# noveens/reviews4rec

Hardware: AMD Instinct MI355X
Metric: train ratings/sec (higher is better)
Workload: dtype f32

## Files before the change

include/r4r.h:

```cpp
#ifndef R4R_H
#define R4R_H

#include <stddef.h>
#include <stdint.h>

#ifdef __cplusplus
extern "C" {
#endif

#define R4R_OK 0
#define R4R_ERR_ARG (-1)
#define R4R_ERR_LAUNCH (-2)
#define R4R_ERR_WORKSPACE (-3)

int r4r_version(void);
const char *r4r_last_error(void);

size_t r4r_textcnn_ws_bytes(int64_t N, int T, int E, int F, int64_t V);
int r4r_textcnn_fwd(const float *table, int64_t V, const int64_t *idx,
                    const float *conv_w, const float *conv_b,
                    float *pooled, int32_t *argmax,
                    void *ws, size_t ws_bytes,
                    int64_t N, int T, int E, int F, void *stream);

int r4r_conv_algo(int requested, int64_t N, int T, int E, int F);

int r4r_textcnn_algo(int requested);

int r4r_conv_pick(int E, int T, int64_t docs, int64_t rows, int64_t V);

int r4r_gemm_math(int mode, float table_maxabs, float weight_maxabs);

int r4r_gemm_form(int balanced);

int r4r_textcnn_wgrad(const float *table, int64_t V, const int64_t *idx,
                      const float *g_pooled, const int32_t *argmax,
                      float *d_conv_w, float *d_conv_b,
                      void *ws, size_t ws_bytes,
                      int64_t N, int T, int E, int F, void *stream);

int r4r_linear_fwd(const float *x, const float *w, const float *b, float *y,
                   int64_t N, int n_in, int n_out, int relu, void *stream);
size_t r4r_linear_bwd_ws_bytes(int64_t N, int n_in, int n_out);
int r4r_linear_bwd(const float *x, const float *w, const float *y, const float *g_y,
                   float *g_x, float *g_w, float *g_b, void *ws, size_t ws_bytes,
                   int64_t N, int n_in, int n_out, int relu, void *stream);

int r4r_dropout_fwd(const float *x, float *y, float *mult, int64_t n, float p,
                    uint64_t seed, uint64_t offset, uint64_t *offset_dev, void *stream);
int r4r_counter_add(uint64_t *counter, uint64_t delta, void *stream);
int r4r_mul(const float *a, const float *b, float *out, int64_t n, void *stream);
int r4r_add(const float *a, const float *b, float *out, int64_t n, void *stream);

int r4r_fm_fwd(const float *x, const float *V, const float *lin_w, const float *lin_b,
               float *out, int64_t N, int n, int k, void *stream);
int r4r_fm_bwd(const float *x, const float *V, const float *lin_w, const float *g_out,
// ... 45 lines not shown
                      float weight_decay, int64_t step, void *stream);
int r4r_adam_gathered_guarded(float *p, const float *gathered, int world, float *g_sum, float *m, float *v,
                              int64_t numel, float lr, double beta1, double beta2, float eps,
                              float weight_decay, int64_t step, const uint32_t *abort_word, void *stream);

int r4r_peer_segment_create(int64_t bytes, void **ptr, uint8_t *handle);
int r4r_peer_segment_open(const uint8_t *handle, void **ptr);
int r4r_peer_segment_close(void *ptr);
int r4r_peer_segment_destroy(void *ptr);
int r4r_peer_push(const float *src, int64_t numel, const uint64_t *peer_dst, const uint64_t *peer_flags,
                  uint32_t *arrive, int rank, int world, uint32_t epoch, const uint32_t *wait_flags,
                  uint32_t *timed_out, double timeout_s, void *stream);
int r4r_peer_wait(const uint32_t *flags, int world, uint32_t epoch, uint32_t *timed_out, double timeout_s, void *stream);


#define R4R_CONV_AUTO 0
#define R4R_CONV_DIRECT 1
#define R4R_CONV_PROJECT 2
int r4r_deepconn_nparam(void);
int r4r_deepconn_layout(int E, int L, int64_t *offsets, int64_t *sizes, int64_t *total);
size_t r4r_deepconn_ws_bytes(int64_t B, int T, int E, int L, int64_t V);
size_t r4r_deepconn_ws_mult_offset(int64_t B, int T, int E, int L, int64_t V);
size_t r4r_deepconn_ws_count_offset(int64_t B, int T, int E, int L, int64_t V, int tower, int buffer);
int r4r_deepconn_step(const float *table, int64_t V, const int64_t *user_idx, const int64_t *item_idx,
                      const float *y, float *flat_p, float *flat_g,
                      float *pred, float *se, float *sse_accum,
                      void *ws, size_t ws_bytes,
                      int64_t B, int T, int E, int L,
                      float dropout_p, int training, uint64_t seed, uint64_t offset,
                      float inv_denom, int conv_algo, int token_buffer, int tokens_ready,
                      const int64_t *next_user_idx, const int64_t *next_item_idx,
                      float *flat_m, float *flat_v, float lr, double beta1, double beta2, float eps,
                      float weight_decay, int64_t adam_step, void *stream);
int r4r_deepconn_tokens(const int64_t *user_idx, const int64_t *item_idx, void *ws, size_t ws_bytes,
                        int64_t B, int T, int E, int L, int64_t V, int conv_algo, int token_buffer,
                        int discard, void *stream);

#define R4R_TIMING_TEXTCNN_FWD 0
#define R4R_TIMING_TEXTCNN_WGRAD 1
#define R4R_TIMING_ADAM 2
#define R4R_TIMING_PROJ_GEMM 3
#define R4R_TIMING_PROJ_GATHER 4
#define R4R_TIMING_SLOTS 8
int r4r_timing_enable(int slot_mask);
int r4r_timing_read(int slot, double *total_ms, int64_t *count, int reset);

// ... 365 lines not shown
```

reviews4rec_amd/csrc/engine.hip:

```cpp
#include <stdlib.h>

#include "trace_device.h"
#include "textcnn.h"
#include "wgrad_device.h"
#include "tokens_device.h"
#include "adam_device.h"

namespace r4r {

constexpr int F_CONV = 100;
constexpr int FM_K = 8;
constexpr int MAX_L = 128;

enum { P_UCW = 0, P_UCB, P_UFW, P_UFB, P_ICW, P_ICB, P_IFW, P_IFB, P_FMV, P_FMLW, P_FMLB, P_GB, P_COUNT };

struct Layout {
    int64_t off[P_COUNT], size[P_COUNT], total;
};

static Layout make_layout(int E, int L) {
    Layout lay;
    const int64_t sz[P_COUNT] = {(int64_t)F_CONV * 3 * E, F_CONV, (int64_t)L * F_CONV, L,
                                 (int64_t)F_CONV * 3 * E, F_CONV, (int64_t)L * F_CONV, L,
                                 (int64_t)2 * L * FM_K, 2 * L, 1, 1};
// ... 1 lines not shown
    for (int i = 0; i < P_COUNT; ++i) {
        lay.off[i] = o;
        lay.size[i] = sz[i];
        o += (sz[i] + 31) & ~(int64_t)31;
    }
    lay.total = o;
    return lay;
}

struct HeadArgs {
    const float *pmax[2]; const int *parg[2];
    const float *fc_w[2]; const float *fc_b[2];
    const float *V, *lin_w, *lin_b, *gbias;
    const float *y;
    float *pooled[2]; int *argmax[2];
    float *g_pooled[2];
    float *mult;
    float *x, *s, *g, *gz;
    float *pred, *se;
    int64_t B;
    int L, tiles, training, want_grad;
    float p_drop, inv_denom;
    uint64_t seed, offset;
};


constexpr int HEAD_MAX_TILES = 8;

#define SEL2(arr, s) ((s) ? (arr)[1] : (arr)[0])
HEAD_TRACE_DEFINE(r4r_debug_dc_head_trace)
template <int ML>
__global__ __launch_bounds__(256) void deepconn_head_wg_kernel(HeadArgs a) {
    HEAD_STAMP(0)
    constexpr int N2 = 2 * ML, PARTS = 256 / N2;
    __shared__ float sw[2][ML][F_CONV + 1];
    __shared__ float sfb[N2], slw[N2], sz[N2];
    __shared__ float sV[N2][FM_K];
    __shared__ float sp[2][F_CONV + 4];
    __shared__ float red[N2][PARTS + 1];
    const int tid = threadIdx.x, lane = tid & 63, w = tid >> 6;
    const int64_t b = blockIdx.x;
    const int L = a.L, n = 2 * L;
    const float lin_b0 = a.lin_b[0], gbias0 = a.gbias[0], yb = a.y ? a.y[b] : 0.f;

    constexpr int FQ = F_CONV / 4;
    typedef float hq4 __attribute__((ext_vector_type(4)));
    constexpr int WREGS = (2 * ML * FQ + 255) / 256;
    hq4 wreg[WREGS];
    const int wtot = 2 * L * FQ;
#pragma unroll
    for (int k = 0; k < WREGS; ++k) {
        const int i = min(tid + 256 * k, wtot - 1);
        const int t = i >= L * FQ;
        wreg[k] = *reinterpret_cast<const hq4 *>(SEL2(a.fc_w, t) + 4 * (i - t * L * FQ));
    }
    const int tn = min(tid, n - 1);
    const float fbreg = SEL2(a.fc_b, tn >= L)[tn - (tn >= L ? L : 0)];
    const float lwreg = a.lin_w[tn];
    constexpr int VREGS = (N2 * FM_K + 255) / 256;
    float vreg[VREGS];
#pragma unroll
    for (int k = 0; k < VREGS; ++k) vreg[k] = a.V[min(tid + 256 * k, n * FM_K - 1)];

    {
        const int t = w >> 1, f = lane + 64 * (w & 1), fc = min(f, F_CONV - 1);
        float best = -INFINITY;
        int bp = -1;
        if (a.tiles <= HEAD_MAX_TILES) {
            float v[HEAD_MAX_TILES];
            int pp[HEAD_MAX_TILES];
#pragma unroll
            for (int k = 0; k < HEAD_MAX_TILES; ++k) {
                const size_t o = ((size_t)b * a.tiles + min(k, a.tiles - 1)) * NP + fc;
                v[k] = SEL2(a.pmax, t)[o];
                pp[k] = SEL2(a.parg, t)[o];
            }
#pragma unroll
            for (int k = 0; k < HEAD_MAX_TILES; ++k)
                if (v[k] > best) { best = v[k]; bp = pp[k]; }
        } else {
            for (int k0 = 0; k0 < a.tiles; k0 += HEAD_MAX_TILES) {
                float v[HEAD_MAX_TILES];
                int pp[HEAD_MAX_TILES];
#pragma unroll
                for (int k = 0; k < HEAD_MAX_TILES; ++k) {
// ... 195 lines not shown
        float t = 0.f;
#pragma unroll
        for (int r = 0; r < HG_ROWS; ++r) t += red[r][ox];
        switch (which) {
            case 0: a.g_fc_w[0][local] = t; break;
            case 1: a.g_fc_b[0][local] = t; break;
            case 2: a.g_fc_w[1][local] = t; break;
            case 3: a.g_fc_b[1][local] = t; break;
            case 4: a.g_V[local] = t; break;
            case 5: a.g_lin_w[local] = t; break;
            case 6: a.g_lin_b[0] = t; break;
            case 7: a.g_gb[0] = t; break;
            default: if (a.sse_accum) a.sse_accum[0] += t; break;
        }
    }
}

BWD_TRACE_DEFINE(r4r_debug_dc_bwd_trace)
struct DcBackwardArgs {
    WgradArgs w;
    HeadGradArgs h;
    int hg_blocks;
    TokenArgs nx;
};
__global__ __launch_bounds__(WG_THREADS, 8) void deepconn_backward_kernel(DcBackwardArgs) {
    const DcBackwardArgs &A = kernel_args<DcBackwardArgs>();
    const WgradArgs &w = A.w;
    const HeadGradArgs &h = A.h;
    const TokenArgs &nx = A.nx;
    const int hg_blocks = A.hg_blocks;
    BWD_STAMP(0, wall_clock64())
    BWD_STAMP(2, (unsigned long long)blockIdx.z + 1)
    if (blockIdx.z == 1 || blockIdx.z == 2) {
        wgrad_block(w, blockIdx.x, blockIdx.y, blockIdx.z - 1);
    } else if (blockIdx.z == 0) {
        for (int blk = blockIdx.y * gridDim.x + blockIdx.x; blk < hg_blocks; blk += gridDim.x * gridDim.y) {
            head_grad_block(h, blk);
            __syncthreads();
        }
    } else {
        token_mark_block(nx, blockIdx.y * gridDim.x + blockIdx.x, gridDim.x * gridDim.y, WG_THREADS);
    }
#ifdef R4R_TRACE
    __syncthreads();
#endif
    BWD_STAMP(1, wall_clock64())
}

constexpr int RED_THREADS = 256;
struct FusedAdam {
    float *p, *m, *v;
    const float *g;
    int64_t lo[2], hi[2];
    AdamScalars s;
    int on;
};
__global__ __launch_bounds__(RED_THREADS) void deepconn_reduce_kernel(WgradArgs w, int red_blocks, int comp_blocks,
                                                                      TokenArgs nx, FusedAdam opt) {
    const int bx = blockIdx.x;
    if (bx < red_blocks) {
        const WgradTower &tw = w.t[blockIdx.y];
        const int nw = w.F * 3 * w.E;
        const int i = bx * RED_THREADS + threadIdx.x;
        const float *gp0 = i < nw ? tw.d_w + i : (i < nw + w.F ? tw.d_b + (i - nw) : nullptr);
// ... 14 lines not shown
            float P = opt.p[o], M = opt.m[o], V = opt.v[o];
            adam_elem(P, opt.g[o], M, V, opt.s);
            opt.p[o] = P; opt.m[o] = M; opt.v[o] = V;
        }
    }
}

__global__ void sse_only_kernel(const float *__restrict__ se, float *__restrict__ accum, int64_t B) {
    __shared__ float red[256];
    float s = 0.f;
    for (int64_t i = threadIdx.x; i < B; i += 256) s += se[i];
    red[threadIdx.x] = s;
    __syncthreads();
    for (int off = 128; off > 0; off >>= 1) {
        if ((int)threadIdx.x < off) red[threadIdx.x] += red[threadIdx.x + off];
        __syncthreads();
    }
    if (threadIdx.x == 0) accum[0] += red[0];
}

struct StepWs {
    float *wp[2], *pmax[2]; int *parg[2];
    int *flags[2][2], *slot[2][2], *list[2][2], *count[2][2]; float *ptab[2];
    float *pooled[2]; int *argmax[2]; float *g_pooled[2];
    float *mult, *x, *s, *g, *gz;
    float *part_w[2], *part_b[2];
    size_t bytes;
};

static StepWs carve(void *ws, int64_t B, int T, int E, int L, int64_t V) {
    StepWs w;
    char *p = static_cast<char *>(ws);
    auto take = [&](size_t nbytes) { char *r = p; p += align256(nbytes); return r; };
    const size_t tiles128 = (size_t)(T + 2 + 127) / 128;
    const int ns = textcnn_wgrad_splits(B);
    for (int t = 0; t < 2; ++t) {
        w.wp[t] = reinterpret_cast<float *>(take(textcnn_wp_floats(E) * 4));
        w.pmax[t] = reinterpret_cast<float *>(take((size_t)B * tiles128 * NP * 4));
        w.parg[t] = reinterpret_cast<int *>(take((size_t)B * tiles128 * NP * 4));
        w.pooled[t] = reinterpret_cast<float *>(take((size_t)B * F_CONV * 4));
        w.argmax[t] = reinterpret_cast<int *>(take((size_t)B * F_CONV * 4));
        w.g_pooled[t] = reinterpret_cast<float *>(take((size_t)B * F_CONV * 4));
        w.part_w[t] = reinterpret_cast<float *>(take((size_t)ns * F_CONV * 3 * E * 4));
        w.part_b[t] = reinterpret_cast<float *>(take((size_t)ns * F_CONV * 4));
        for (int bf = 0; bf < 2; ++bf) {
            w.flags[bf][t] = reinterpret_cast<int *>(take((size_t)(V + 4) * 4));
            w.slot[bf][t] = reinterpret_cast<int *>(take((size_t)(V + 4) * 4));
            w.list[bf][t] = reinterpret_cast<int *>(take((size_t)proj_row_capacity(B, T, V) * 4));
            w.count[bf][t] = reinterpret_cast<int *>(take(256));
        }
        w.ptab[t] = reinterpret_cast<float *>(take(proj_ptab_floats(B, T, V) * 4));
    }
    w.mult = reinterpret_cast<float *>(take((size_t)B * 2 * L * 4));
    w.x = reinterpret_cast<float *>(take((size_t)B * 2 * L * 4));
    w.gz = reinterpret_cast<float *>(take((size_t)B * 2 * L * 4));
    w.s = reinterpret_cast<float *>(take((size_t)B * FM_K * 4));
    w.g = reinterpret_cast<float *>(take((size_t)B * 4));
    w.bytes = (size_t)(p - static_cast<char *>(ws));
    return w;
}

}

using namespace r4r;

extern "C" int r4r_deepconn_nparam(void) { return P_COUNT; }

extern "C" int r4r_deepconn_layout(int E, int L, int64_t *offsets, int64_t *sizes, int64_t *total) {
    R4R_REQUIRE(E > 0 && L > 0 && L <= MAX_L && offsets && sizes && total, "deepconn_layout: bad arguments");
    const Layout lay = make_layout(E, L);
    for (int i = 0; i < P_COUNT; ++i) { offsets[i] = lay.off[i]; sizes[i] = lay.size[i]; }
    *total = lay.total;
    return R4R_OK;
}

extern "C" size_t r4r_deepconn_ws_bytes(int64_t B, int T, int E, int L, int64_t V) {
    if (B < 0 || T <= 0 || E <= 0 || L <= 0 || V <= 0) return 0;
    return carve(nullptr, B, T, E, L, V).bytes;
}

extern "C" size_t r4r_deepconn_ws_mult_offset(int64_t B, int T, int E, int L, int64_t V) {
    char base[1];
    const StepWs w = carve(base, B, T, E, L, V);
    return (size_t)(reinterpret_cast<char *>(w.mult) - base);
}

extern "C" size_t r4r_deepconn_ws_count_offset(int64_t B, int T, int E, int L, int64_t V, int tower, int buffer) {
    char base[1];
    const StepWs w = carve(base, B, T, E, L, V);
    return (size_t)(reinterpret_cast<char *>(w.count[buffer & 1][tower & 1]) - base);
}

extern "C" int r4r_deepconn_tokens(const int64_t *user_idx, const int64_t *item_idx, void *ws, size_t ws_bytes,
                                   int64_t B, int T, int E, int L, int64_t V, int conv_algo, int token_buffer,
                                   int discard, void *stream) {
    R4R_REQUIRE(user_idx && item_idx && ws, "deepconn_tokens: null pointer");
    R4R_REQUIRE(token_buffer == 0 || token_buffer == 1, "deepconn_tokens: token_buffer must be 0 or 1");
    if (ws_bytes < r4r_deepconn_ws_bytes(B, T, E, L, V)) {
        set_error("deepconn_tokens: workspace %zu < %zu bytes", ws_bytes, r4r_deepconn_ws_bytes(B, T, E, L, V));
        return R4R_ERR_WORKSPACE;
    }
    if (B == 0 || textcnn_pick_algo(conv_algo, B, T, E, F_CONV) != R4R_CONV_PROJECT) return R4R_OK;
    const StepWs w = carve(ws, B, T, E, L, V);
    if (discard) {
        for (int t = 0; t < 2; ++t) (void)hipMemsetAsync(w.count[token_buffer][t], 0, sizeof(int), as_stream(stream));
        return check_launch("deepconn_tokens(discard)");
    }
    ProjTower pt[2];
    const int64_t *idx[2] = {user_idx, item_idx};
    for (int t = 0; t < 2; ++t) {
        pt[t] = ProjTower{};
        pt[t].idx = idx[t];
        pt[t].flags = w.flags[token_buffer][t]; pt[t].slot = w.slot[token_buffer][t];
        pt[t].list = w.list[token_buffer][t]; pt[t].count = w.count[token_buffer][t];
    }
    return textcnn_proj_tokens_launch(V, pt, 2, B, T, false, as_stream(stream));
}

extern "C" int r4r_deepconn_step(const float *table, int64_t V, const int64_t *user_idx, const int64_t *item_idx,
                                 const float *y, float *flat_p, float *flat_g,
                                 float *pred, float *se, float *sse_accum,
                                 void *ws, size_t ws_bytes,
                                 int64_t B, int T, int E, int L,
                                 float dropout_p, int training, uint64_t seed, uint64_t offset,
                                 float inv_denom, int conv_algo, int token_buffer, int tokens_ready,
                                 const int64_t *next_user_idx, const int64_t *next_item_idx,
                                 float *flat_m, float *flat_v, float lr, double beta1, double beta2, float eps,
                                 float weight_decay, int64_t adam_step,
// ... 20 lines not shown
    if (B == 0) return R4R_OK;
    hipStream_t st = as_stream(stream);
    const Layout lay = make_layout(E, L);
    const StepWs w = carve(ws, B, T, E, L, V);
    const float *P[P_COUNT];
    float *G[P_COUNT];
    for (int i = 0; i < P_COUNT; ++i) {
        P[i] = flat_p + lay.off[i];
        G[i] = flat_g ? flat_g + lay.off[i] : nullptr;
    }

    const int64_t *idx[2] = {user_idx, item_idx};
    const int algo = textcnn_pick_algo(conv_algo, B, T, E, F_CONV);
    int tiles;
    if (algo == R4R_CONV_PROJECT) {
        ProjTower pt[2];
        for (int t = 0; t < 2; ++t) {
            pt[t].idx = idx[t];
            pt[t].conv_w = P[t ? P_ICW : P_UCW];
            pt[t].conv_b = P[t ? P_ICB : P_UCB];
            pt[t].flags = w.flags[token_buffer][t]; pt[t].slot = w.slot[token_buffer][t];
            pt[t].list = w.list[token_buffer][t]; pt[t].count = w.count[token_buffer][t];
            pt[t].ptab = w.ptab[t]; pt[t].pmax = w.pmax[t]; pt[t].parg = w.parg[t]; pt[t].wimg = w.wp[t];
        }
        if (!tokens_ready)
            if (int rc = textcnn_proj_tokens_launch(V, pt, 2, B, T, false, st)) return rc;
        if (int rc = textcnn_proj_compute_launch(table, V, pt, 2, B, T, E, F_CONV, st)) return rc;
        tiles = proj_tiles(T);
    } else {
        FwdTower ft[2];
        for (int t = 0; t < 2; ++t) {
            ft[t].idx = idx[t];
            ft[t].conv_w = P[t ? P_ICW : P_UCW];
            ft[t].conv_b = P[t ? P_ICB : P_UCB];
            ft[t].wp = w.wp[t]; ft[t].pmax = w.pmax[t]; ft[t].parg = w.parg[t];
        }
        if (int rc = textcnn_fwd_launch(table, ft, 2, B, T, E, F_CONV, st)) return rc;
        tiles = textcnn_tiles(T);
    }

    HeadArgs h;
    for (int t = 0; t < 2; ++t) {
        h.pmax[t] = w.pmax[t]; h.parg[t] = w.parg[t];
        h.fc_w[t] = P[t ? P_IFW : P_UFW]; h.fc_b[t] = P[t ? P_IFB : P_UFB];
        h.pooled[t] = w.pooled[t]; h.argmax[t] = w.argmax[t]; h.g_pooled[t] = w.g_pooled[t];
    }
    h.V = P[P_FMV]; h.lin_w = P[P_FMLW]; h.lin_b = P[P_FMLB]; h.gbias = P[P_GB];
    h.y = y; h.mult = w.mult; h.x = w.x; h.s = w.s; h.g = w.g; h.gz = w.gz;
    h.pred = pred; h.se = se;
    h.B = B; h.L = L; h.tiles = tiles; h.training = training; h.want_grad = flat_g != nullptr;
    h.p_drop = dropout_p; h.inv_denom = inv_denom; h.seed = seed; h.offset = offset;
    if (L <= 16) deepconn_head_wg_kernel<16><<<(unsigned)B, 256, 0, st>>>(h);
    else if (L <= 32) deepconn_head_wg_kernel<32><<<(unsigned)B, 256, 0, st>>>(h);
    else if (L <= 64) deepconn_head_wg_kernel<64><<<(unsigned)B, 256, 0, st>>>(h);
    else deepconn_head_wg_kernel<128><<<(unsigned)B, 256, 0, st>>>(h);

    if (!flat_g) {
        if (y && sse_accum) sse_only_kernel<<<1, 256, 0, st>>>(se, sse_accum, B);
        return check_launch("deepconn_step(forward)");
    }

    HeadGradArgs hg;
    for (int t = 0; t < 2; ++t) {
        hg.pooled[t] = w.pooled[t];
        hg.g_fc_w[t] = G[t ? P_IFW : P_UFW]; hg.g_fc_b[t] = G[t ? P_IFB : P_UFB];
    }
    hg.x = w.x; hg.s = w.s; hg.g = w.g; hg.gz = w.gz; hg.V = P[P_FMV]; hg.se = se;
    hg.g_V = G[P_FMV]; hg.g_lin_w = G[P_FMLW]; hg.g_lin_b = G[P_FMLB]; hg.g_gb = G[P_GB];
    hg.sse_accum = sse_accum; hg.B = B; hg.L = L;
    const int nout = 2 * (L * F_CONV + L) + 2 * L * FM_K + 2 * L + 3;
    const int hg_blocks = (nout + HG_COLS - 1) / HG_COLS;

    WgradTower wt[2];
    WgradArgs wa;
    for (int t = 0; t < 2; ++t) {
        wt[t].idx = idx[t]; wt[t].g_pooled = w.g_pooled[t]; wt[t].argmax = w.argmax[t];
        wt[t].part_w = w.part_w[t]; wt[t].part_b = w.part_b[t];
        wt[t].d_w = G[t ? P_ICW : P_UCW]; wt[t].d_b = G[t ? P_ICB : P_UCB];
    }
    for (int k = 0; k < MAX_TOWERS; ++k) wa.t[k] = wt[k < 2 ? k : 0];
    wa.table = table; wa.N = B; wa.T = T; wa.E = E; wa.F = F_CONV;
    wa.table_bytes = (int64_t)V * E * 4;
    wa.nsplit = textcnn_wgrad_splits(B);
    wa.per_split = (int)cdiv(B, wa.nsplit);
    const bool prefetch = next_user_idx && algo == R4R_CONV_PROJECT;
    TokenArgs nx{};
    if (prefetch) {
        ProjTower nt[2];
        const int64_t *nidx[2] = {next_user_idx, next_item_idx};
        const int ob = token_buffer ^ 1;
        for (int t = 0; t < 2; ++t) {
            nt[t] = ProjTower{};
            nt[t].idx = nidx[t];
            nt[t].flags = w.flags[ob][t]; nt[t].slot = w.slot[ob][t];
            nt[t].list = w.list[ob][t]; nt[t].count = w.count[ob][t];
        }
        nx = make_token_args(V, nt, 2, B, T);
    }
    {
        ScopedTiming tm(R4R_TIMING_TEXTCNN_WGRAD, st);
        deepconn_backward_kernel<<<dim3(F_CONV, wa.nsplit, prefetch ? 4 : 3), WG_THREADS, 0, st>>>(DcBackwardArgs{wa, hg, hg_blocks, nx});
    }
    const int red_blocks = (F_CONV * 3 * E + F_CONV + RED_THREADS - 1) / RED_THREADS;
    const int comp_blocks = prefetch ? (int)cdiv((V + 3) / 4, RED_THREADS * compact_groups(V)) : 0;
    FusedAdam opt{};
    int opt_blocks = 0;
    if (flat_m) {
        opt.on = 1;
        opt.p = flat_p; opt.m = flat_m; opt.v = flat_v; opt.g = flat_g;
        opt.lo[0] = lay.off[P_UFW]; opt.hi[0] = lay.off[P_ICW];
        opt.lo[1] = lay.off[P_IFW]; opt.hi[1] = lay.total;
        opt.s = adam_make_scalars(lr, beta1, beta2, eps, weight_decay, adam_step, nullptr);
        const int64_t longest = opt.hi[0] - opt.lo[0] > opt.hi[1] - opt.lo[1] ? opt.hi[0] - opt.lo[0] : opt.hi[1] - opt.lo[1];
        opt_blocks = (int)cdiv(longest, RED_THREADS);
    }
    deepconn_reduce_kernel<<<dim3(red_blocks + comp_blocks + opt_blocks, 2), RED_THREADS, 0, st>>>(
        wa, red_blocks, comp_blocks, nx, opt);
    return check_launch("deepconn_step");
}

extern "C" int r4r_sse_accumulate(const float *se, int64_t n, float *accum, void *stream) {
    R4R_REQUIRE(accum && (se || n == 0) && n >= 0, "sse_accumulate: bad arguments");
    if (n == 0) return R4R_OK;
    sse_only_kernel<<<1, 256, 0, as_stream(stream)>>>(se, accum, n);
// ... 3 lines not shown
```

reviews4rec_amd/csrc/project.hip:

```cpp
#include <stdlib.h>

#include <type_traits>

#include "textcnn.h"
#include "tokens_device.h"
#include "trace_device.h"

namespace r4r {

typedef float f32x4 __attribute__((ext_vector_type(4)));

constexpr int PF = 100;
constexpr int PROW = 3 * PF;
#ifndef R4R_PSTR
#define R4R_PSTR 304
#endif
constexpr int PSTR = R4R_PSTR;
static_assert(PSTR >= PROW && PSTR % 4 == 0, "projected-row stride");
constexpr int PN = 304;
constexpr int PNT = PN / 16;
constexpr int PEC = 16;
constexpr int PS = PEC + 8;
constexpr int GM = 2;
constexpr int PM = 64 * GM;
// ... 985 lines not shown

constexpr int SLICE = 32;
constexpr int GWPS = SEG / SLICE;
constexpr int GSPW = 8 / GWPS;
static_assert(SLICE == 32 || SLICE == 16, "a worker is 32 lanes; eight workers per workgroup");
constexpr int GATHER_ROTDIV = 16;
constexpr int GDEPTH = 7;

HEAD_TRACE_DEFINE(r4r_debug_gather_trace)
__global__ __launch_bounds__(256) void proj_gather_max_kernel(ProjArgs a) {
    HEAD_STAMP(0)
    __shared__ int sl[8][SLICE + 2];
    __shared__ float sbest[8][PF];
    __shared__ int sbp[8][PF];
    const ProjTower &tw = a.t[blockIdx.y];
    const int worker = threadIdx.x >> 5, wl = threadIdx.x & 31;
    unsigned bx = blockIdx.x;
    if (GSPW == 2 && (a.tiles & 1) == 0 && a.tiles >= 4) {
        const unsigned t2 = (unsigned)a.tiles >> 1;
        const unsigned d = bx / t2, pr = bx - d * t2;
        bx = d * t2 + (pr + d / GATHER_ROTDIV) % t2;
    }
    const unsigned units = (unsigned)(a.N * a.tiles);
    auto unit_of = [&](int h) -> unsigned { return bx * GSPW + h; };
    const unsigned unit = unit_of(worker / GWPS);
    const unsigned udoc = unit < units ? unit / (unsigned)a.tiles : 0u;
    const int64_t doc = udoc;
    const int seg = unit < units ? (int)(unit - udoc * (unsigned)a.tiles) : a.tiles;
    const int T = a.T, P = T + 2;
    const bool act = wl < PF / 4;
    const f32x4 zero = (f32x4){0.f, 0.f, 0.f, 0.f};
    if (blockIdx.x == 0 && threadIdx.x == 0) {
        tw.count[1] = tw.count[0];
        tw.count[0] = 0;
    }

#ifndef R4R_GATHER_EVEN_SLICES
#define R4R_GATHER_EVEN_SLICES 1
#endif
    const int seg_len = min(SEG, P - seg * SEG);
    const int slen = (R4R_GATHER_EVEN_SLICES && seg_len > 0 && seg_len < SEG) ? (seg_len + GWPS - 1) / GWPS : SLICE;
    const int p_lo = seg * SEG + (worker % GWPS) * slen;
    const int p_hi = min(min(P, (seg + 1) * SEG), p_lo + slen);
    const int t_lo = p_lo - 2;
    const int ntok = (seg < a.tiles && p_hi > p_lo) ? p_hi - t_lo : 0;
    bool same = true;
    {
        const int ta = t_lo + wl, tb = t_lo + 32 + wl;
        const bool va = wl < ntok && ta >= 0 && ta < T, vb = 32 + wl < ntok && tb >= 0 && tb < T;
        int64_t ia = tw.idx[doc * T + (va ? ta : 0)], ib = tw.idx[doc * T + (vb ? tb : 0)];
        asm volatile("" : "+v"(ia), "+v"(ib));
        const int sa = tw.slot[ia], sb = tw.slot[ib];
        if (wl < ntok) sl[worker][wl] = va ? sa : -1;
        if (32 + wl < ntok) sl[worker][32 + wl] = vb ? sb : -1;
    }
    __syncthreads();
    HEAD_STAMP(1)
    if (ntok > 0) {
        const int s_first = sl[worker][0];
        for (int k = wl; k < ntok; k += 32) same &= (sl[worker][k] == s_first);
    }
    {
        const unsigned long long m = __ballot(same);
        const unsigned long long mine = (worker & 1) ? (m >> 32) : (m & 0xffffffffull);
        same = (mine == 0xffffffffull);
    }
    const int npos_eff = same ? min(1, ntok - 2) : ntok - 2;

    float best[4] = {-INFINITY, -INFINITY, -INFINITY, -INFINITY};
    int bp[4] = {0x7fffffff, 0x7fffffff, 0x7fffffff, 0x7fffffff};
    if (ntok > 0 && act) {
        const f32x4 bias = *reinterpret_cast<const f32x4 *>(tw.conv_b + wl * 4);
        const float *base = tw.ptab + wl * 4;
        f32x4 s_a = zero, s_b = zero;
// ... 22 lines not shown
                if (k + u < npos) {
                    const int p = p_lo + k + u;
                    const f32x4 y = (s_a + r2[u]) + bias;
#pragma unroll
                    for (int c = 0; c < 4; ++c)
                        if (y[c] > best[c]) { best[c] = y[c]; bp[c] = p; }
                    s_a = s_b + r1[u];
                    s_b = r0[u];
                }
            }
        };
        for (int k = 0; k < npos; k += GDEPTH) {
            f32x4 r0[GDEPTH], r1[GDEPTH], r2[GDEPTH];
            loadg(k, r0, r1, r2);
            compg(k, r0, r1, r2);
        }
    }
    if (act) {
#pragma unroll
        for (int c = 0; c < 4; ++c) { sbest[worker][wl * 4 + c] = best[c]; sbp[worker][wl * 4 + c] = bp[c]; }
    }
    __syncthreads();
    HEAD_STAMP(2)
    const int half = threadIdx.x >> 7, f = threadIdx.x & 127;
    const unsigned ounit = unit_of(half);
    if (f < PF && ounit < units && half < GSPW) {
        float mb = sbest[half * GWPS][f];
        int mp = sbp[half * GWPS][f];
#pragma unroll
        for (int w = 1; w < GWPS; ++w) {
            const float v = sbest[half * GWPS + w][f];
            if (v > mb) { mb = v; mp = sbp[half * GWPS + w][f]; }
        }
        const size_t o = (size_t)ounit * NP + f;
        tw.pmax[o] = mb;
        tw.parg[o] = mp;
    }
    HEAD_STAMP(3)
}

int proj_tiles(int T) { return (T + 2 + SEG - 1) / SEG; }
int64_t proj_row_capacity(int64_t N, int T, int64_t V) { return (N * T < V) ? N * T : V; }
size_t proj_ptab_floats(int64_t N, int T, int64_t V) { return (size_t)proj_row_capacity(N, T, V) * PSTR; }

constexpr int GEMM_DEFAULT_FORM = 5;
constexpr int WR_DEFAULT_CHUNKS = 4;
static int g_gemm_balanced = -1;
static int g_gemm_math = 0;
static float g_table_maxabs = 0.f;
static float g_weight_maxabs = 0.f;
int proj_gemm_f16_launch(const float *table, const ProjTower *tw, int ntower, int cap, int E, float table_maxabs,
                         float weight_maxabs, hipStream_t st);
size_t proj_gemm_f16_wimg_bytes(int E);

static ProjArgs make_args(const float *table, int64_t V, const ProjTower *tw, int ntower,
// ... 75 lines not shown
        ScopedTiming tm(R4R_TIMING_PROJ_GEMM, st);
        if (int rc = proj_gemm_f16_launch(table, tw, ntower, a.cap, E, g_table_maxabs, g_weight_maxabs, st)) return rc;
    } else if (a.balanced == 4) {
        int64_t wgs = ((int64_t)a.cap + 15) / 16 * WR_NQ / WR_WAVES + ntower;
        const int64_t resident = (int64_t)G7_WGS * (wgs >= 8 * G7_WGS ? wr_wgs_per_cu(a.nchunk) : 1);
        if (wgs > resident) wgs = resident;
        if (wgs < ntower) wgs = ntower;
        wres_launch(a, (unsigned)wgs, st);
    } else {
        const int rows_wg = (a.balanced == 3 ? AR_PMIN : G7_ROWS) * 16;
        int64_t wgs = ((int64_t)a.cap + rows_wg - 1) / rows_wg * ntower;
        if (wgs > G7_WGS) wgs = G7_WGS;
        const int ares_bytes = a.nchunk * AR_CHUNK * 4;
        const int lds_bytes = (a.balanced == 3 && ares_bytes > GEMM_LDS_BYTES) ? ares_bytes : GEMM_LDS_BYTES;
        launch_timed(R4R_TIMING_PROJ_GEMM, proj_gemm_kernel, dim3((unsigned)wgs), dim3(GEMM_THREADS), lds_bytes, st, a);
    }
    {
        ScopedTiming tm(R4R_TIMING_PROJ_GATHER, st, true);
        proj_gather_max_kernel<<<dim3((unsigned)cdiv(N * a.tiles, GSPW), ntower), 256, 0, st>>>(a);
    }
    return check_launch("textcnn_proj_fwd");
}

void proj_gemm_set_form(int balanced) { g_gemm_balanced = balanced; }
int proj_gemm_math_mode() { return g_gemm_math; }
void proj_gemm_set_math(int mode, float table_maxabs, float weight_maxabs) {
    g_gemm_math = mode; g_table_maxabs = table_maxabs; g_weight_maxabs = weight_maxabs;
}

int textcnn_proj_fwd_launch(const float *table, int64_t V, const ProjTower *tw, int ntower,
                            int64_t N, int T, int E, int F, bool zero_state, hipStream_t st) {
    if (int rc = textcnn_proj_tokens_launch(V, tw, ntower, N, T, zero_state, st)) return rc;
    return textcnn_proj_compute_launch(table, V, tw, ntower, N, T, E, F, st);
}

}
```

reviews4rec_amd/csrc/textcnn.h:

```cpp
#pragma once
#include "common.h"

namespace r4r {

constexpr int NP = 112;
constexpr int MAX_TOWERS = 4;

struct FwdTower {
    const int64_t *idx;
    const float *conv_w;
    const float *conv_b;
    float *wp;
    float *pmax;
    int *parg;
};

struct WgradTower {
    const int64_t *idx;
    const float *g_pooled;
    const int *argmax;
    float *part_w;
    float *part_b;
    float *d_w;
    float *d_b;
};

struct ProjTower {
    const int64_t *idx;
    const float *conv_w;
    const float *conv_b;
    int *flags;
    int *slot;
    int *list;
    int *count;
    float *ptab;
    float *pmax;
    int *parg;
    float *wimg = nullptr;
};
int proj_tiles(int T);
int64_t proj_row_capacity(int64_t N, int T, int64_t V);
size_t proj_ptab_floats(int64_t N, int T, int64_t V);
int textcnn_proj_fwd_launch(const float *table, int64_t V, const ProjTower *tw, int ntower,
                            int64_t N, int T, int E, int F, bool zero_state, hipStream_t st);
int textcnn_proj_tokens_launch(int64_t V, const ProjTower *tw, int ntower, int64_t N, int T,
                               bool zero_state, hipStream_t st);
int textcnn_proj_compute_launch(const float *table, int64_t V, const ProjTower *tw, int ntower,
                                int64_t N, int T, int E, int F, hipStream_t st);
void proj_gemm_set_math(int mode, float table_maxabs, float weight_maxabs);
int proj_gemm_math_mode();
void proj_gemm_set_form(int balanced);
int textcnn_pick_algo(int requested, int64_t N, int T, int E, int F);

size_t textcnn_wp_floats(int E);
int textcnn_tile_rows(int T);
int textcnn_tiles(int T);
int textcnn_wgrad_splits(int64_t N);

int textcnn_fwd_launch(const float *table, const FwdTower *tw, int ntower,
                       int64_t N, int T, int E, int F, hipStream_t st);
int textcnn_pool_finish_launch(const float *pmax, const int *parg, float *pooled, int *argmax,
                               int64_t N, int tiles, int F, hipStream_t st);
int textcnn_wgrad_launch(const float *table, const WgradTower *tw, int ntower,
                         int64_t N, int T, int E, int F, hipStream_t st, int64_t table_bytes = 0);

int textcnn_wgrad_reduce_launch(const WgradTower *tw, int ntower, int64_t N, int E, int F, hipStream_t st);

static inline size_t align256(size_t x) { return (x + 255) & ~(size_t)255; }

}
```

reviews4rec_amd/csrc/textcnn.hip:

```cpp
#include <stdlib.h>

#include <math.h>
#include "textcnn.h"
#include "wgrad_device.h"

namespace r4r {

typedef float f32x4 __attribute__((ext_vector_type(4)));

constexpr int NT = NP / 16;
constexpr int EC = 16;
constexpr int XS = EC + 8;
constexpr int WS = 3 * EC + 8;
constexpr int W_VEC = NP * WS / 4;

template <int NW>
struct Cfg {
    static constexpr int THREADS = 64 * NW;
    static constexpr int MTILE = 32 * NW;
    static constexpr int XROWS = MTILE + 2;
    static constexpr int BUF_FLOATS = XROWS * XS + NP * WS;
    static constexpr int LDS_BYTES = 2 * BUF_FLOATS * 4;
    static constexpr int XK = MTILE * 4 / THREADS;
    static constexpr int WK = (W_VEC + THREADS - 1) / THREADS;
// ... 392 lines not shown
    const int64_t tiles = (rows + 127) / 128 + 1, tail = tiles % 256;
    const double round = 11.0 + 0.14 * E;
    const double last = tail == 0 ? 0.0 : (tail * 4 <= 256 ? 9.3 + 0.044 * E : (tail * 2 <= 256 ? 13.8 + 0.071 * E : round));
    const double t_gemm = (double)(tiles / 256) * round + last;
    double t_gather = (double)docs * P * (0.085 + 0.0006 * ((double)rows * 1200.0 / 1e6)) * 1e-3;
    if (t_gather < 10.0) t_gather = 10.0;
    const double t_tokens = 4.0 + 0.027 * ((double)V / 1000.0);
    return (t_gemm + t_gather + t_tokens < t_direct) ? R4R_CONV_PROJECT : R4R_CONV_DIRECT;
}

extern "C" int r4r_gemm_math(int mode, float table_maxabs, float weight_maxabs) {
    R4R_REQUIRE(mode >= 0 && mode <= 2, "gemm_math: mode %d (0 fp32, 1 f16x2 in the fused steps, 2 also in r4r_textcnn_fwd)", mode);
    R4R_REQUIRE(mode == 0 || (table_maxabs > 0.f && table_maxabs < 3.0e38f && weight_maxabs > 0.f && weight_maxabs < 3.0e38f),
                "gemm_math: f16x2 needs max |table| > 0 and max |conv weights| > 0");
    proj_gemm_set_math(mode, table_maxabs, weight_maxabs);
    return R4R_OK;
}

extern "C" int r4r_gemm_form(int balanced) {
    proj_gemm_set_form(balanced);
    return R4R_OK;
}

extern "C" int r4r_textcnn_wgrad(const float *table, int64_t V, const int64_t *idx,
                                 const float *g_pooled, const int32_t *argmax,
                                 float *d_conv_w, float *d_conv_b,
                                 void *ws, size_t ws_bytes,
                                 int64_t N, int T, int E, int F, void *stream) {
    if (int rc = check_tower_args(table, V, idx, N, T, E, F)) return rc;
    R4R_REQUIRE(g_pooled && argmax && d_conv_w && d_conv_b && ws, "textcnn_wgrad: null pointer");
    if (ws_bytes < r4r_textcnn_ws_bytes(N, T, E, F, V)) {
        set_error("textcnn_wgrad: workspace %zu < %zu bytes", ws_bytes, r4r_textcnn_ws_bytes(N, T, E, F, V));
        return R4R_ERR_WORKSPACE;
    }
    const int ns = textcnn_wgrad_splits(N);
    char *base = static_cast<char *>(ws);
    WgradTower tw;
    tw.idx = idx; tw.g_pooled = g_pooled; tw.argmax = argmax; tw.d_w = d_conv_w; tw.d_b = d_conv_b;
    tw.part_w = reinterpret_cast<float *>(base);
    base += align256((size_t)ns * F * 3 * E * 4);
    tw.part_b = reinterpret_cast<float *>(base);
    const char *rows = getenv("R4R_WGRAD_ROWS");
    const bool loop = rows && rows[0] == 'l';
    return textcnn_wgrad_launch(table, &tw, 1, N, T, E, F, as_stream(stream), loop ? 0 : (int64_t)V * E * 4);
}
```

reviews4rec_amd/csrc/tokens_device.h:

```cpp
#pragma once
#include "textcnn.h"

namespace r4r {

struct TokenTower {
    const int64_t *idx;
    int *flags, *slot, *list, *count;
};
struct TokenArgs {
    TokenTower t[MAX_TOWERS];
    int64_t N, V;
    int T, ntower;
};

__device__ __forceinline__ void token_mark_block(const TokenArgs &a, int blk, int nblk, int nthreads) {
    const int64_t total = a.N * a.T;
    for (int t = 0; t < a.ntower; ++t) {
        const int64_t *__restrict__ idx = a.t[t].idx;
        int *__restrict__ flags = a.t[t].flags;
        for (int64_t i = (int64_t)blk * nthreads + threadIdx.x; i < total; i += (int64_t)nblk * nthreads)
            flags[idx[i]] = 1;
    }
}

// ... 35 lines not shown
        const int64_t gi = g0 + (int64_t)g * (64 * NW);
        if (gi >= ngroups) continue;
        int at = base_row + wsum[g * NW + wave] + incl[g] - cnt[g];
        const int fl[4] = {f[g].x, f[g].y, f[g].z, f[g].w};
        int sl[4];
#pragma unroll
        for (int k = 0; k < 4; ++k) {
            sl[k] = -1;
            if (fl[k]) { sl[k] = at; tw.list[at] = (int)(gi * 4 + k); ++at; }
        }
        *reinterpret_cast<int4 *>(tw.slot + gi * 4) = make_int4(sl[0], sl[1], sl[2], sl[3]);
        if (cnt[g]) reinterpret_cast<int4 *>(tw.flags)[gi] = make_int4(0, 0, 0, 0);
    }
}
constexpr int COMPACT_BIG_G = 8;
constexpr int64_t COMPACT_BIG_V = 262144;
static inline int compact_groups(int64_t V) { return V > COMPACT_BIG_V ? COMPACT_BIG_G : 1; }
template <int NW>
__device__ __forceinline__ void token_compact_auto(const TokenTower &tw, int64_t V, int blk) {
    if (V > COMPACT_BIG_V) token_compact_block<NW, COMPACT_BIG_G>(tw, V, blk);
    else token_compact_block<NW, 1>(tw, V, blk);
}

static inline TokenArgs make_token_args(int64_t V, const ProjTower *tw, int ntower, int64_t N, int T) {
    TokenArgs a;
    for (int k = 0; k < MAX_TOWERS; ++k) {
        const ProjTower &s = tw[k < ntower ? k : 0];
        a.t[k].idx = s.idx; a.t[k].flags = s.flags; a.t[k].slot = s.slot; a.t[k].list = s.list; a.t[k].count = s.count;
    }
    a.N = N; a.V = V; a.T = T; a.ntower = ntower;
    return a;
}

}
```

Measured before the change: 1.388 million.

## Plan gather work order by segment liveness for next batch's projection gather

Extra head-kernel workgroups scan the next batch's token segments and flag those containing more than one distinct token. The backward kernel then compacts the flags into a permutation. When enough segments are uniform (padding), the gather kernel pairs a live segment with a uniform one in each workgroup, aiming to balance load across workgroups. This adds planning work, extra workspace, and cross-kernel readiness flags that can be reset or reused incorrectly.

```diff
diff --git a/include/r4r.h b/include/r4r.h
--- a/include/r4r.h
+++ b/include/r4r.h
@@ -32,6 +32,8 @@
 int r4r_gemm_math(int mode, float table_maxabs, float weight_maxabs);
 
 int r4r_gemm_form(int balanced);
+
+int r4r_gather_plan(int on);
 
 int r4r_textcnn_wgrad(const float *table, int64_t V, const int64_t *idx,
                       const float *g_pooled, const int32_t *argmax,
@@ -123,6 +125,8 @@
 size_t r4r_deepconn_ws_bytes(int64_t B, int T, int E, int L, int64_t V);
 size_t r4r_deepconn_ws_mult_offset(int64_t B, int T, int E, int L, int64_t V);
 size_t r4r_deepconn_ws_count_offset(int64_t B, int T, int E, int L, int64_t V, int tower, int buffer);
+size_t r4r_deepconn_ws_partials_offset(int64_t B, int T, int E, int L, int64_t V, int tower, int which);
+size_t r4r_deepconn_ws_plan_offset(int64_t B, int T, int E, int L, int64_t V, int tower, int buffer, int which);
 int r4r_deepconn_step(const float *table, int64_t V, const int64_t *user_idx, const int64_t *item_idx,
                       const float *y, float *flat_p, float *flat_g,
                       float *pred, float *se, float *sse_accum,
diff --git a/reviews4rec_amd/csrc/engine.hip b/reviews4rec_amd/csrc/engine.hip
--- a/reviews4rec_amd/csrc/engine.hip
+++ b/reviews4rec_amd/csrc/engine.hip
@@ -47,6 +47,8 @@
     int L, tiles, training, want_grad;
     float p_drop, inv_denom;
     uint64_t seed, offset;
+    PlanArgs plan;
+    int *plan_spent[2];
 };
 
 
@@ -56,6 +58,10 @@
 HEAD_TRACE_DEFINE(r4r_debug_dc_head_trace)
 template <int ML>
 __global__ __launch_bounds__(256) void deepconn_head_wg_kernel(HeadArgs a) {
+    if ((int64_t)blockIdx.x >= a.B) {
+        segment_flags_wave(a.plan, ((int)blockIdx.x - (int)a.B) * 4 + (int)(threadIdx.x >> 6));
+        return;
+    }
     HEAD_STAMP(0)
     constexpr int N2 = 2 * ML, PARTS = 256 / N2;
     __shared__ float sw[2][ML][F_CONV + 1];
@@ -86,6 +92,7 @@
     float vreg[VREGS];
 #pragma unroll
     for (int k = 0; k < VREGS; ++k) vreg[k] = a.V[min(tid + 256 * k, n * FM_K - 1)];
+    if (b == 0 && tid < 2 && SEL2(a.plan_spent, tid)) SEL2(a.plan_spent, tid)[0] = 0;
 
     {
         const int t = w >> 1, f = lane + 64 * (w & 1), fc = min(f, F_CONV - 1);
@@ -327,12 +334,14 @@
     HeadGradArgs h;
     int hg_blocks;
     TokenArgs nx;
+    PlanArgs plan;
 };
 __global__ __launch_bounds__(WG_THREADS, 8) void deepconn_backward_kernel(DcBackwardArgs) {
     const DcBackwardArgs &A = kernel_args<DcBackwardArgs>();
     const WgradArgs &w = A.w;
     const HeadGradArgs &h = A.h;
     const TokenArgs &nx = A.nx;
+    const PlanArgs &plan = A.plan;
     const int hg_blocks = A.hg_blocks;
     BWD_STAMP(0, wall_clock64())
     BWD_STAMP(2, (unsigned long long)blockIdx.z + 1)
@@ -344,7 +353,9 @@
             __syncthreads();
         }
     } else {
-        token_mark_block(nx, blockIdx.y * gridDim.x + blockIdx.x, gridDim.x * gridDim.y, WG_THREADS);
+        const int np = plan.units > 0 ? 2 : 0, blk = blockIdx.y * gridDim.x + blockIdx.x;
+        if (blk < np) segment_plan_block<WG_THREADS>(plan, blk);
+        else token_mark_block(nx, blk - np, gridDim.x * gridDim.y - np, WG_THREADS);
     }
 #ifdef R4R_TRACE
     __syncthreads();
@@ -405,6 +416,7 @@
 struct StepWs {
     float *wp[2], *pmax[2]; int *parg[2];
     int *flags[2][2], *slot[2][2], *list[2][2], *count[2][2]; float *ptab[2];
+    int *live[2][2], *perm[2][2], *plan_ready[2][2];
     float *pooled[2]; int *argmax[2]; float *g_pooled[2];
     float *mult, *x, *s, *g, *gz;
     float *part_w[2], *part_b[2];
@@ -439,6 +451,12 @@
     w.gz = reinterpret_cast<float *>(take((size_t)B * 2 * L * 4));
     w.s = reinterpret_cast<float *>(take((size_t)B * FM_K * 4));
     w.g = reinterpret_cast<float *>(take((size_t)B * 4));
+    for (int t = 0; t < 2; ++t)
+        for (int bf = 0; bf < 2; ++bf) {
+            w.live[bf][t] = reinterpret_cast<int *>(take((size_t)PLAN_MAX_UNITS * 4));
+            w.perm[bf][t] = reinterpret_cast<int *>(take((size_t)PLAN_MAX_UNITS * 4));
+            w.plan_ready[bf][t] = reinterpret_cast<int *>(take(256));
+        }
     w.bytes = (size_t)(p - static_cast<char *>(ws));
     return w;
 }
@@ -472,6 +490,25 @@
     char base[1];
     const StepWs w = carve(base, B, T, E, L, V);
     return (size_t)(reinterpret_cast<char *>(w.count[buffer & 1][tower & 1]) - base);
+}
+
+extern "C" size_t r4r_deepconn_ws_partials_offset(int64_t B, int T, int E, int L, int64_t V, int tower, int which) {
+    char base[1];
+    const StepWs w = carve(base, B, T, E, L, V);
+    const void *at = which ? static_cast<const void *>(w.parg[tower & 1]) : w.pmax[tower & 1];
+    return (size_t)(static_cast<const char *>(at) - base);
+}
+extern "C" size_t r4r_deepconn_ws_plan_offset(int64_t B, int T, int E, int L, int64_t V, int tower, int buffer, int which) {
+    char base[1];
+    const StepWs w = carve(base, B, T, E, L, V);
+    const int t = tower & 1, bf = buffer & 1;
+    const void *at[3] = {w.perm[bf][t], w.plan_ready[bf][t], w.live[bf][t]};
+    return (which < 0 || which > 2) ? 0 : (size_t)(static_cast<const char *>(at[which]) - base);
+}
+
+static bool plan_applies(int64_t B, int T) {
+    const int tiles = proj_tiles(T);
+    return proj_gather_plan() && (tiles & 1) == 0 && B * tiles <= PLAN_MAX_UNITS;
 }
 
 extern "C" int r4r_deepconn_tokens(const int64_t *user_idx, const int64_t *item_idx, void *ws, size_t ws_bytes,
@@ -486,7 +523,10 @@
     if (B == 0 || textcnn_pick_algo(conv_algo, B, T, E, F_CONV) != R4R_CONV_PROJECT) return R4R_OK;
     const StepWs w = carve(ws, B, T, E, L, V);
     if (discard) {
-        for (int t = 0; t < 2; ++t) (void)hipMemsetAsync(w.count[token_buffer][t], 0, sizeof(int), as_stream(stream));
+        for (int t = 0; t < 2; ++t) {
+            (void)hipMemsetAsync(w.count[token_buffer][t], 0, sizeof(int), as_stream(stream));
+            (void)hipMemsetAsync(w.plan_ready[token_buffer][t], 0, sizeof(int), as_stream(stream));
+        }
         return check_launch("deepconn_tokens(discard)");
     }
     ProjTower pt[2];
@@ -553,6 +593,9 @@
             pt[t].flags = w.flags[token_buffer][t]; pt[t].slot = w.slot[token_buffer][t];
             pt[t].list = w.list[token_buffer][t]; pt[t].count = w.count[token_buffer][t];
             pt[t].ptab = w.ptab[t]; pt[t].pmax = w.pmax[t]; pt[t].parg = w.parg[t]; pt[t].wimg = w.wp[t];
+            if (tokens_ready && plan_applies(B, T)) {
+                pt[t].perm = w.perm[token_buffer][t]; pt[t].plan_ready = w.plan_ready[token_buffer][t];
+            }
         }
         if (!tokens_ready)
             if (int rc = textcnn_proj_tokens_launch(V, pt, 2, B, T, false, st)) return rc;
@@ -581,10 +624,23 @@
     h.pred = pred; h.se = se;
     h.B = B; h.L = L; h.tiles = tiles; h.training = training; h.want_grad = flat_g != nullptr;
     h.p_drop = dropout_p; h.inv_denom = inv_denom; h.seed = seed; h.offset = offset;
-    if (L <= 16) deepconn_head_wg_kernel<16><<<(unsigned)B, 256, 0, st>>>(h);
-    else if (L <= 32) deepconn_head_wg_kernel<32><<<(unsigned)B, 256, 0, st>>>(h);
-    else if (L <= 64) deepconn_head_wg_kernel<64><<<(unsigned)B, 256, 0, st>>>(h);
-    else deepconn_head_wg_kernel<128><<<(unsigned)B, 256, 0, st>>>(h);
+    const bool planning = next_user_idx && flat_g && algo == R4R_CONV_PROJECT && plan_applies(B, T);
+    PlanArgs plan{};
+    if (planning) {
+        const int ob = token_buffer ^ 1;
+        plan.idx[0] = next_user_idx; plan.idx[1] = next_item_idx;
+        for (int t = 0; t < 2; ++t) {
+            plan.live[t] = w.live[ob][t]; plan.perm[t] = w.perm[ob][t]; plan.plan_ready[t] = w.plan_ready[ob][t];
+        }
+        plan.T = T; plan.tiles = proj_tiles(T); plan.units = (int)(B * plan.tiles);
+    }
+    h.plan = plan;
+    for (int t = 0; t < 2; ++t) h.plan_spent[t] = algo == R4R_CONV_PROJECT ? w.plan_ready[token_buffer][t] : nullptr;
+    const unsigned head_wgs = (unsigned)B + (unsigned)cdiv(2 * (int64_t)plan.units, 4);
+    if (L <= 16) deepconn_head_wg_kernel<16><<<head_wgs, 256, 0, st>>>(h);
+    else if (L <= 32) deepconn_head_wg_kernel<32><<<head_wgs, 256, 0, st>>>(h);
+    else if (L <= 64) deepconn_head_wg_kernel<64><<<head_wgs, 256, 0, st>>>(h);
+    else deepconn_head_wg_kernel<128><<<head_wgs, 256, 0, st>>>(h);
 
     if (!flat_g) {
         if (y && sse_accum) sse_only_kernel<<<1, 256, 0, st>>>(se, sse_accum, B);
@@ -630,7 +686,7 @@
     }
     {
         ScopedTiming tm(R4R_TIMING_TEXTCNN_WGRAD, st);
-        deepconn_backward_kernel<<<dim3(F_CONV, wa.nsplit, prefetch ? 4 : 3), WG_THREADS, 0, st>>>(DcBackwardArgs{wa, hg, hg_blocks, nx});
+        deepconn_backward_kernel<<<dim3(F_CONV, wa.nsplit, prefetch ? 4 : 3), WG_THREADS, 0, st>>>(DcBackwardArgs{wa, hg, hg_blocks, nx, plan});
     }
     const int red_blocks = (F_CONV * 3 * E + F_CONV + RED_THREADS - 1) / RED_THREADS;
     const int comp_blocks = prefetch ? (int)cdiv((V + 3) / 4, RED_THREADS * compact_groups(V)) : 0;
diff --git a/reviews4rec_amd/csrc/project.hip b/reviews4rec_amd/csrc/project.hip
--- a/reviews4rec_amd/csrc/project.hip
+++ b/reviews4rec_amd/csrc/project.hip
@@ -1031,14 +1031,20 @@
         bx = d * t2 + (pr + d / GATHER_ROTDIV) % t2;
     }
     const unsigned units = (unsigned)(a.N * a.tiles);
-    auto unit_of = [&](int h) -> unsigned { return bx * GSPW + h; };
-    const unsigned unit = unit_of(worker / GWPS);
-    const unsigned udoc = unit < units ? unit / (unsigned)a.tiles : 0u;
-    const int64_t doc = udoc;
-    const int seg = unit < units ? (int)(unit - udoc * (unsigned)a.tiles) : a.tiles;
+    const int half = worker / GWPS;
+    unsigned unit = bx * GSPW + half;
     const int T = a.T, P = T + 2;
     const bool act = wl < PF / 4;
     const f32x4 zero = (f32x4){0.f, 0.f, 0.f, 0.f};
+    int plan_word = 0;
+    unsigned punit = 0;
+    if (GSPW == 2 && tw.perm) {
+        typedef const int __attribute__((address_space(1))) *global_int;
+        global_int ready = (global_int)tw.plan_ready;
+        asm volatile("" : "+v"(ready));
+        plan_word = ready[0];
+        punit = (unsigned)tw.perm[half ? units - 1 - blockIdx.x : blockIdx.x];
+    }
     if (blockIdx.x == 0 && threadIdx.x == 0) {
         tw.count[1] = tw.count[0];
         tw.count[0] = 0;
@@ -1047,18 +1053,34 @@
 #ifndef R4R_GATHER_EVEN_SLICES
 #define R4R_GATHER_EVEN_SLICES 1
 #endif
-    const int seg_len = min(SEG, P - seg * SEG);
-    const int slen = (R4R_GATHER_EVEN_SLICES && seg_len > 0 && seg_len < SEG) ? (seg_len + GWPS - 1) / GWPS : SLICE;
-    const int p_lo = seg * SEG + (worker % GWPS) * slen;
-    const int p_hi = min(min(P, (seg + 1) * SEG), p_lo + slen);
-    const int t_lo = p_lo - 2;
-    const int ntok = (seg < a.tiles && p_hi > p_lo) ? p_hi - t_lo : 0;
+    int64_t doc;
+    int p_lo, p_hi, t_lo, ntok;
+    bool va, vb;
+    int64_t ia, ib;
+    auto place = [&]() {
+        const unsigned udoc = unit < units ? unit / (unsigned)a.tiles : 0u;
+        doc = udoc;
+        const int seg = unit < units ? (int)(unit - udoc * (unsigned)a.tiles) : a.tiles;
+        const int seg_len = min(SEG, P - seg * SEG);
+        const int slen = (R4R_GATHER_EVEN_SLICES && seg_len > 0 && seg_len < SEG) ? (seg_len + GWPS - 1) / GWPS : SLICE;
+        p_lo = seg * SEG + (worker % GWPS) * slen;
+        p_hi = min(min(P, (seg + 1) * SEG), p_lo + slen);
+        t_lo = p_lo - 2;
+        ntok = (seg < a.tiles && p_hi > p_lo) ? p_hi - t_lo : 0;
+        const int ta = t_lo + wl, tb = t_lo + 32 + wl;
+        va = wl < ntok && ta >= 0 && ta < T; vb = 32 + wl < ntok && tb >= 0 && tb < T;
+        ia = tw.idx[doc * T + (va ? ta : 0)]; ib = tw.idx[doc * T + (vb ? tb : 0)];
+        asm volatile("" : "+v"(ia), "+v"(ib));
+    };
+    place();
+    const int planned = __builtin_amdgcn_readfirstlane(plan_word);
+    if (planned) {
+        unit = punit;
+        place();
+    }
+    if (blockIdx.x == 0 && threadIdx.x == 0 && tw.perm) tw.count[2] = planned ? 1 : 0;
     bool same = true;
     {
-        const int ta = t_lo + wl, tb = t_lo + 32 + wl;
-        const bool va = wl < ntok && ta >= 0 && ta < T, vb = 32 + wl < ntok && tb >= 0 && tb < T;
-        int64_t ia = tw.idx[doc * T + (va ? ta : 0)], ib = tw.idx[doc * T + (vb ? tb : 0)];
-        asm volatile("" : "+v"(ia), "+v"(ib));
         const int sa = tw.slot[ia], sb = tw.slot[ib];
         if (wl < ntok) sl[worker][wl] = va ? sa : -1;
         if (32 + wl < ntok) sl[worker][32 + wl] = vb ? sb : -1;
@@ -1127,15 +1149,15 @@
     }
     __syncthreads();
     HEAD_STAMP(2)
-    const int half = threadIdx.x >> 7, f = threadIdx.x & 127;
-    const unsigned ounit = unit_of(half);
-    if (f < PF && ounit < units && half < GSPW) {
-        float mb = sbest[half * GWPS][f];
-        int mp = sbp[half * GWPS][f];
+    const int mhalf = threadIdx.x >> 7, f = threadIdx.x & 127;
+    const unsigned ounit = unit;
+    if (f < PF && ounit < units && mhalf < GSPW) {
+        float mb = sbest[mhalf * GWPS][f];
+        int mp = sbp[mhalf * GWPS][f];
 #pragma unroll
         for (int w = 1; w < GWPS; ++w) {
-            const float v = sbest[half * GWPS + w][f];
-            if (v > mb) { mb = v; mp = sbp[half * GWPS + w][f]; }
+            const float v = sbest[mhalf * GWPS + w][f];
+            if (v > mb) { mb = v; mp = sbp[mhalf * GWPS + w][f]; }
         }
         const size_t o = (size_t)ounit * NP + f;
         tw.pmax[o] = mb;
@@ -1257,6 +1279,9 @@
     return check_launch("textcnn_proj_fwd");
 }
 
+static int g_gather_plan = 1;
+void proj_gather_set_plan(int on) { g_gather_plan = on ? 1 : 0; }
+int proj_gather_plan() { return g_gather_plan; }
 void proj_gemm_set_form(int balanced) { g_gemm_balanced = balanced; }
 int proj_gemm_math_mode() { return g_gemm_math; }
 void proj_gemm_set_math(int mode, float table_maxabs, float weight_maxabs) {
diff --git a/reviews4rec_amd/csrc/textcnn.h b/reviews4rec_amd/csrc/textcnn.h
--- a/reviews4rec_amd/csrc/textcnn.h
+++ b/reviews4rec_amd/csrc/textcnn.h
@@ -37,6 +37,8 @@
     float *pmax;
     int *parg;
     float *wimg = nullptr;
+    const int *perm = nullptr;
+    const int *plan_ready = nullptr;
 };
 int proj_tiles(int T);
 int64_t proj_row_capacity(int64_t N, int T, int64_t V);
@@ -49,6 +51,8 @@
                                 int64_t N, int T, int E, int F, hipStream_t st);
 void proj_gemm_set_math(int mode, float table_maxabs, float weight_maxabs);
 int proj_gemm_math_mode();
+void proj_gather_set_plan(int on);
+int proj_gather_plan();
 void proj_gemm_set_form(int balanced);
 int textcnn_pick_algo(int requested, int64_t N, int T, int E, int F);
 
diff --git a/reviews4rec_amd/csrc/textcnn.hip b/reviews4rec_amd/csrc/textcnn.hip
--- a/reviews4rec_amd/csrc/textcnn.hip
+++ b/reviews4rec_amd/csrc/textcnn.hip
@@ -438,6 +438,12 @@
     return R4R_OK;
 }
 
+extern "C" int r4r_gather_plan(int on) {
+    const int before = proj_gather_plan();
+    proj_gather_set_plan(on);
+    return before;
+}
+
 extern "C" int r4r_textcnn_wgrad(const float *table, int64_t V, const int64_t *idx,
                                  const float *g_pooled, const int32_t *argmax,
                                  float *d_conv_w, float *d_conv_b,
diff --git a/reviews4rec_amd/csrc/tokens_device.h b/reviews4rec_amd/csrc/tokens_device.h
--- a/reviews4rec_amd/csrc/tokens_device.h
+++ b/reviews4rec_amd/csrc/tokens_device.h
@@ -81,6 +81,89 @@
     else token_compact_block<NW, 1>(tw, V, blk);
 }
 
+constexpr int PLAN_SEG = 128;
+constexpr int PLAN_MAX_UNITS = 4096;
+struct PlanArgs {
+    const int64_t *idx[2];
+    int *live[2];
+    int *perm[2];
+    int *plan_ready[2];
+    int T, tiles, units;
+};
+
+__device__ __forceinline__ void segment_flags_wave(const PlanArgs &p, int g) {
+    const int lane = threadIdx.x & 63;
+    const int t = g >= p.units, u = g - t * p.units;
+    if (u >= p.units) return;
+    const int doc = u / p.tiles, seg = u - doc * p.tiles, T = p.T;
+    const int t_lo = PLAN_SEG * seg - 2, t_hi = min(T + 2, PLAN_SEG * (seg + 1));
+    const int64_t *__restrict__ row = (t ? p.idx[1] : p.idx[0]) + (int64_t)doc * T;
+    long long v[3];
+    bool valid[3], in[3];
+#pragma unroll
+    for (int k = 0; k < 3; ++k) {
+        const int tk = t_lo + 64 * k + lane;
+        valid[k] = tk < t_hi && (k < 2 || lane < 2);
+        in[k] = valid[k] && tk >= 0 && tk < T;
+        v[k] = row[in[k] ? tk : 0];
+    }
+    bool differs = false;
+    long long first = in[0] ? v[0] : -1;
+    first = __shfl(first, 0);
+#pragma unroll
+    for (int k = 0; k < 3; ++k) differs |= valid[k] && (in[k] ? v[k] : -1) != first;
+    if (__ballot(differs) != 0ull && lane == 0) (t ? p.live[1] : p.live[0])[u] = 1;
+}
+
+template <int NT>
+__device__ __forceinline__ void segment_plan_block(const PlanArgs &p, int t) {
+    constexpr int K = PLAN_MAX_UNITS / NT, NW = NT / 64;
+    static_assert(K % 4 == 0 && NT % 64 == 0, "int4 loads of whole waves");
+    __shared__ int wtot[NW];
+    const int tid = threadIdx.x, lane = tid & 63, wave = tid >> 6, units = p.units;
+    int *__restrict__ live = t ? p.live[1] : p.live[0];
+    int *__restrict__ perm = t ? p.perm[1] : p.perm[0];
+    int f[K];
+#pragma unroll
+    for (int q = 0; q < K / 4; ++q) {
+        const int4 x = reinterpret_cast<const int4 *>(live)[tid * (K / 4) + q];
+        f[4 * q] = x.x; f[4 * q + 1] = x.y; f[4 * q + 2] = x.z; f[4 * q + 3] = x.w;
+    }
+    int cnt = 0;
+#pragma unroll
+    for (int k = 0; k < K; ++k) {
+        f[k] = (f[k] != 0 && tid * K + k < units) ? 1 : 0;
+        cnt += f[k];
+    }
+    int incl = cnt;
+#pragma unroll
+    for (int off = 1; off < 64; off <<= 1) {
+        const int up = __shfl_up(incl, off);
+        if (lane >= off) incl += up;
+    }
+    if (lane == 63) wtot[wave] = incl;
+    __syncthreads();
+    int before = incl - cnt, nlive = 0;
+#pragma unroll
+    for (int w = 0; w < NW; ++w) {
+        const int c = wtot[w];
+        if (w < wave) before += c;
+        nlive += c;
+    }
+#pragma unroll
+    for (int k = 0; k < K; ++k) {
+        const int u = tid * K + k;
+        if (u < units) perm[f[k] ? before : nlive + (u - before)] = u;
+        before += f[k];
+    }
+    if (cnt) {
+#pragma unroll
+        for (int q = 0; q < K / 4; ++q) reinterpret_cast<int4 *>(live)[tid * (K / 4) + q] = make_int4(0, 0, 0, 0);
+    }
+    __syncthreads();
+    if (tid == 0) (t ? p.plan_ready[1] : p.plan_ready[0])[0] = ((units - nlive) * 8 >= units) ? 1 : 0;
+}
+
 static inline TokenArgs make_token_args(int64_t V, const ProjTower *tw, int ntower, int64_t N, int T) {
     TokenArgs a;
     for (int k = 0; k < MAX_TOWERS; ++k) {
```

Measured after the change: 1.408 million (median of 6 runs). 1.5% higher.
